# lim271/MultiOutputIHGP

Hardware: AMD Instinct MI355X
Metric: Kalman steps/sec (M outputs x T ticks) + NLL rel-err vs CPU oracle (higher is better)
Workload: dtype f32; 1 GPU; C3-filter: M=L=4096/GPU, T=10000, Matern-5/2 (matern52ss.h, d=3), fp32, filter+NLL; latents_per_gpu=4096, latents_total=4096, ticks=10000, state_dim=3, layout=segment-major [ceil(T/SEG)][L][SEG], SEG = 4 KB of ticks, HBM-resident

## Files before the change

multioutputihgp_amd/csrc/recursion.hip:

```cpp
#include "kernels_common.h"
#include <hip/hip_ext.h>

#ifndef MOIHGP_GENERIC_UNROLL
#define MOIHGP_GENERIC_UNROLL 4
#endif

namespace moihgp {
namespace {

template <typename T, int D, int CK>
struct FastConst {
    T a[D * D];
    T k[D];
    T g[CK * D];
    const T* sp;
    T pj[D * D];
};

template <typename T, int D, int CK, bool NLL, bool TAIL>
__device__ inline void replay_chunk(T* y, T* xs, const FastConst<T, D, CK>& c, size_t t0, size_t Tlen, double& acc, unsigned& nobs) {
    T part = 0;
#pragma unroll
    for (int k = 0; k < CK; k++) {
        const bool valid = !TAIL || (t0 + k) < Tlen;
// ... 417 lines not shown
            }
#pragma unroll
            for (int i = 0; i < D; i++) cc[i] = (double)read_lane(xs[i], jl);
            if (WRITE) {
#pragma unroll
                for (int k = 0; k < VPL; k++) lds[lane * (VPL + 1) + k] = pack<T>(&y[sg][k * EPV]);
                wave_lds_fence();
                T* po = orow + (size_t)sg * SEG + (size_t)lane * EPV;
#pragma unroll
                for (int i = 0; i < VPL; i++) {
                    const int q = i * 64 + lane;
                    if (sg < nfull || (size_t)sg * SEG + (size_t)q * EPV < Tlen) nt_store(lds[q + q / VPL], reinterpret_cast<V*>(po + (size_t)i * 64 * EPV));
                }
                wave_lds_fence();
            }
        }
    }
#pragma unroll
    for (int i = 0; i < D; i++) xout[i] = (T)cc[i];
    return true;
}

constexpr int kMaxSplit = 8;

template <typename T, int D, int CK, bool WRITE, bool NLL, int MINW, bool SPLIT, int DBG = 0>
__global__ void __launch_bounds__(SPLIT ? 64 * kMaxSplit : 64 * kWavesPerBlock, SPLIT ? 1 : MINW)
filter_scan_kernel(const T* __restrict__ Ty, size_t Ttot, size_t ld, size_t L, const T* __restrict__ cbT,
                   const double* __restrict__ cb64, const T* xin0 , T* x ,
                   T* __restrict__ yhat, double* __restrict__ nll, int nsplit, size_t Tslice,
                   int nbig ,
                   size_t ldo , int team ) {
    using V = typename VecOf<T>::type;
    using Lay = CB<D>;
    constexpr int EPV = 16 / sizeof(T);
    constexpr int VPL = CK / EPV;
    constexpr int NVP = 64 * (VPL + 1);
    static_assert(CK % EPV == 0 && CK <= 16, "CK must be a multiple of 16 bytes and fit the G table");
    extern __shared__ __attribute__((aligned(16))) unsigned char smem[];
    V (*lds_all)[NVP] = reinterpret_cast<V (*)[NVP]>(smem);
    constexpr int CR = D * D + D + 2;
    double (*carry)[CR] = reinterpret_cast<double (*)[CR]>(smem + (size_t)(SPLIT ? nsplit : kWavesPerBlock) * NVP * sizeof(V));

    const int lane = threadIdx.x & 63;
    const int wave = __builtin_amdgcn_readfirstlane(threadIdx.x >> 6);
    const size_t l = SPLIT ? (size_t)blockIdx.x : (size_t)blockIdx.x * kWavesPerBlock + wave;
    if (!SPLIT && l >= L) return;
    const size_t Tsl = SPLIT ? (wave < nbig ? Tslice : Tslice - 64 * CK) : 0;
    const size_t toff = SPLIT ? (wave < nbig ? (size_t)wave * Tslice : (size_t)nbig * Tslice + (size_t)(wave - nbig) * (Tslice - 64 * CK)) : 0;
    const size_t Tlen = SPLIT ? (toff >= Ttot ? 0 : ((Ttot - toff) < Tsl ? (Ttot - toff) : Tsl)) : Ttot;
    V* lds = lds_all[wave];

    const T* cb = cbT + l * Lay::SIZE;
    FastConst<T, D, CK> c;
#pragma unroll
    for (int i = 0; i < D * D; i++) c.a[i] = cb[Lay::A + i];
#pragma unroll
    for (int i = 0; i < D; i++) c.k[i] = cb[Lay::K + i];
#pragma unroll
    for (int i = 0; i < CK * D; i++) c.g[i] = cb[Lay::G + i];
    {
        T* spw = reinterpret_cast<T*>(smem + (size_t)(SPLIT ? nsplit : kWavesPerBlock) * NVP * sizeof(V) +
                                      (SPLIT ? (size_t)nsplit * CR * sizeof(double) : 0)) + (size_t)wave * (4 * D * D);
        if (lane < 4 * D * D) spw[lane] = cb[Lay::SP + lane];
        c.sp = spw;
        wave_lds_fence();
    }
#pragma unroll
    for (int i = 0; i < D * D; i++) c.pj[i] = cb[Lay::PJ + (lane & 15) * D * D + i];

    if (cb[Lay::SCANOK] == T(0)) return;
    const T* row = Ty + l * ld + toff;
    T* orow = WRITE ? yhat + l * ldo + toff : nullptr;
    T xin[D];
    double acc = 0.0;
    unsigned nobs = 0;
    size_t nobs_uniform = 0;

    bool team_done = false;
    if (SPLIT) {
        if (team) {
            unsigned char* tb = smem + (size_t)nsplit * NVP * sizeof(V) + (size_t)nsplit * CR * sizeof(double) + (((size_t)nsplit * 4 * D * D * sizeof(T) + 15) & ~(size_t)15);
            double (*e0all)[D] = reinterpret_cast<double (*)[D]>(tb);
            int* dirty = reinterpret_cast<int*>(tb + (size_t)kTeamMaxSegs * D * sizeof(double));
            if (threadIdx.x == 0) *dirty = 0;
            __syncthreads();
            team_done = team_slice<T, D, CK, WRITE, NLL>(row, orow, Tlen, toff, c, lds, lane, e0all, dirty, xin0 + l * D, xin, acc, nobs, nobs_uniform);
        }
    }
    if (SPLIT && !team_done) {
        if (wave < nsplit - 1) {
            T msl[D * D];
#pragma unroll
            for (int i = 0; i < D; i++) xin[i] = T(0);
            sweep<T, D, CK, false, false, true, 0>(row, nullptr, Tlen, xin, c, cb, lds, lane, acc, nobs, nobs_uniform, msl);
            if (lane == 0) {
#pragma unroll
                for (int i = 0; i < D * D; i++) carry[wave][i] = (double)msl[i];
#pragma unroll
                for (int i = 0; i < D; i++) carry[wave][D * D + i] = (double)xin[i];
            }
        }
        __syncthreads();
        double xc[D];
#pragma unroll
        for (int i = 0; i < D; i++) xc[i] = (double)xin0[l * D + i];
        for (int s = 0; s < wave; s++) {
            double xn[D];
#pragma unroll
            for (int i = 0; i < D; i++) {
                double a = carry[s][D * D + i];
#pragma unroll
                for (int j = 0; j < D; j++) a = fma(carry[s][i * D + j], xc[j], a);
                xn[i] = a;
            }
#pragma unroll
            for (int i = 0; i < D; i++) xc[i] = xn[i];
        }
#pragma unroll
        for (int i = 0; i < D; i++) xin[i] = (T)xc[i];
        acc = 0.0; nobs = 0; nobs_uniform = 0;
        __syncthreads();
    } else if (!SPLIT) {
#pragma unroll
        for (int i = 0; i < D; i++) xin[i] = xin0[l * D + i];
    }

    if (!team_done && (WRITE || NLL || !SPLIT || wave == nsplit - 1)) {
        T unused[D * D];
        sweep<T, D, CK, WRITE, NLL, false, DBG>(row, orow, Tlen, xin, c, cb, lds, lane, acc, nobs, nobs_uniform, unused);
    }

    if (NLL) {
#pragma unroll
        for (int o = 32; o > 0; o >>= 1) {
            acc += __shfl_xor(acc, o);
            nobs += __shfl_xor(nobs, o);
        }
    }
    const double* c64 = cb64 + l * Lay::SIZE;
    if (SPLIT) {
        if (NLL) {
            if (lane == 0) { carry[wave][D * D + D] = acc; carry[wave][D * D + D + 1] = (double)nobs_uniform + (double)nobs; }
            __syncthreads();
        }
        if (lane == 0 && wave == nsplit - 1) {
#pragma unroll
            for (int i = 0; i < D; i++) x[l * D + i] = xin[i];
        }
        if (NLL && lane == 0 && wave == 0) {
            double a = 0.0, n = 0.0;
            for (int s = 0; s < nsplit; s++) { a += carry[s][D * D + D]; n += carry[s][D * D + D + 1]; }
            nll[l] = 0.5 * (a / c64[Lay::S] + n * c64[Lay::LOGS]);
        }
    } else if (lane == 0) {
#pragma unroll
        for (int i = 0; i < D; i++) x[l * D + i] = xin[i];
        if (NLL) {
            double n = (double)nobs_uniform + (double)nobs;
            nll[l] = 0.5 * (acc / c64[Lay::S] + n * c64[Lay::LOGS]);
        }
    }
}

__global__ void __launch_bounds__(1024) nll_total_kernel(const double* __restrict__ nll, size_t L, double* __restrict__ total) {
    __shared__ double red[16];
    const int tid = threadIdx.x, lane = tid & 63, wave = tid >> 6;
    constexpr int kBatch = 8;
    double s = 0.0;
    for (size_t base = 0; base < L; base += (size_t)kBatch * 1024) {
        double v[kBatch];
#pragma unroll
        for (int j = 0; j < kBatch; j++) {
            const size_t i = base + (size_t)j * 1024 + tid;
            const double t = nll[i < L ? i : L - 1];
            v[j] = i < L ? t : 0.0;
        }
#pragma unroll
        for (int j = 0; j < kBatch; j++) s += v[j];
    }
#pragma unroll
    for (int o = 32; o > 0; o >>= 1) s += __shfl_xor(s, o);
    if (lane == 0) red[wave] = s;
    __syncthreads();
    if (tid == 0) {
        double t = 0.0;
        for (int w = 0; w < 16; w++) t += red[w];
        *total = t;
    }
}

template <typename T, int D, bool TILED = false>
__global__ void __launch_bounds__(64)
filter_seq_kernel(const T* __restrict__ Ty, size_t Tlen, size_t ld, size_t L, const T* __restrict__ cbT, const double* __restrict__ cb64,
                  const T* xin0, T* x, T* __restrict__ yhat, double* __restrict__ nll, size_t ldo) {
    using V = typename VecOf<T>::type;
    using Lay = CB<D>;
    constexpr int EPV = 16 / sizeof(T);
    constexpr size_t SEGT = 4096 / sizeof(T);
    auto at = [&](size_t l_, size_t t_, size_t ld_) { return TILED ? ((t_ / SEGT) * L + l_) * SEGT + t_ % SEGT : l_ * ld_ + t_; };
    const size_t l = (size_t)blockIdx.x * blockDim.x + threadIdx.x;
    if (l >= L) return;
    const T* cb = cbT + l * Lay::SIZE;
    if (cb[Lay::SCANOK] != T(0)) return;
    T a[D * D], kk[D], xs[D];
    for (int i = 0; i < D * D; i++) a[i] = cb[Lay::A + i];
    for (int i = 0; i < D; i++) { kk[i] = cb[Lay::K + i]; xs[i] = xin0[l * D + i]; }
    double acc = 0.0, n = 0.0;
    for (size_t tb = 0; tb < Tlen; tb += EPV) {
        T yv[EPV];
        unpack<T>(*reinterpret_cast<const V*>(Ty + at(l, tb, ld)), yv);
        for (int e = 0; e < EPV && tb + e < Tlen; e++) {
            const T yk = yv[e];
            const bool miss = (yk != yk);
            T hx = 0;
            for (int q = 0; q < D; q++) hx = fma(a[q], xs[q], hx);
            const T v = miss ? T(0) : yk - hx;
            if (!miss) { acc = fma((double)v, (double)v, acc); n += 1.0; }
            T xn[D];
            xn[0] = fma(kk[0], v, hx);
            for (int i = 1; i < D; i++) {
                T s = kk[i] * v;
                for (int q = 0; q < D; q++) s = fma(a[i * D + q], xs[q], s);
                xn[i] = s;
            }
            for (int i = 0; i < D; i++) xs[i] = xn[i];
            if (yhat) yhat[at(l, tb + e, ldo)] = xs[0];
        }
    }
    for (int i = 0; i < D; i++) x[l * D + i] = xs[i];
    if (nll) { const double* c64 = cb64 + l * Lay::SIZE; nll[l] = 0.5 * (acc / c64[Lay::S] + n * c64[Lay::LOGS]); }
}

#ifndef MOIHGP_FILTER_DMA
#define MOIHGP_FILTER_DMA 1
#endif
constexpr int kDmaRing32 = 8, kDmaWaves32 = 4;
constexpr int kDmaRing64 = 8, kDmaWaves64 = 3;
typedef __attribute__((address_space(3))) void lds_void_t;
typedef __attribute__((address_space(1))) const void glb_cvoid_t;
__device__ inline unsigned lds_addr_of(const void* p) { return (unsigned)(unsigned long long)(__attribute__((address_space(3))) const char*)p; }
template <int N> __device__ inline void wait_vmcnt() { asm volatile("s_waitcnt vmcnt(%0)" ::"n"(N) : "memory"); }

template <typename T> struct AsmVec;
template <> struct AsmVec<float> { using type = nt_f4; };
template <> struct AsmVec<double> { using type = nt_d2; };
__device__ inline void av_unpack(const nt_f4& v, float* o) { o[0] = v.x; o[1] = v.y; o[2] = v.z; o[3] = v.w; }
__device__ inline void av_unpack(const nt_d2& v, double* o) { o[0] = v.x; o[1] = v.y; }
__device__ inline nt_f4 av_pack(const float* i) { nt_f4 v = {i[0], i[1], i[2], i[3]}; return v; }
__device__ inline nt_d2 av_pack(const double* i) { nt_d2 v = {i[0], i[1]}; return v; }

template <typename AV>
__device__ inline void lds_read4(unsigned a0, unsigned a1, unsigned a2, unsigned a3, AV (&r)[4]) {
    asm volatile("ds_read_b128 %0, %4\n\tds_read_b128 %1, %5\n\tds_read_b128 %2, %6\n\tds_read_b128 %3, %7\n\ts_waitcnt lgkmcnt(0)"
                 : "=&v"(r[0]), "=&v"(r[1]), "=&v"(r[2]), "=&v"(r[3]) : "v"(a0), "v"(a1), "v"(a2), "v"(a3) : "memory");
}
template <typename AV>
__device__ inline void lds_write4(unsigned a0, unsigned a1, unsigned a2, unsigned a3, const AV (&r)[4]) {
    asm volatile("ds_write_b128 %4, %0\n\tds_write_b128 %5, %1\n\tds_write_b128 %6, %2\n\tds_write_b128 %7, %3"
                 :: "v"(r[0]), "v"(r[1]), "v"(r[2]), "v"(r[3]), "v"(a0), "v"(a1), "v"(a2), "v"(a3) : "memory");
}
template <typename AV>
__device__ inline void lds_read4_kb(unsigned a, AV (&r)[4]) {
    asm volatile("ds_read_b128 %0, %4\n\tds_read_b128 %1, %4 offset:1024\n\tds_read_b128 %2, %4 offset:2048\n\tds_read_b128 %3, %4 offset:3072\n\ts_waitcnt lgkmcnt(0)"
                 : "=&v"(r[0]), "=&v"(r[1]), "=&v"(r[2]), "=&v"(r[3]) : "v"(a) : "memory");
}
template <typename T, int N>
__device__ inline void lds_read_uniform(unsigned addr, T* out) {
    using AV = typename AsmVec<T>::type;
    constexpr int EPV = 16 / sizeof(T), NV = (N + EPV - 1) / EPV;
    static_assert(NV >= 1 && NV <= 5, "table row of 1..5 vectors");
    AV v[5];
    if constexpr (NV == 1) asm volatile("ds_read_b128 %0, %1\n\ts_waitcnt lgkmcnt(0)" : "=&v"(v[0]) : "v"(addr) : "memory");
    else if constexpr (NV == 2) asm volatile("ds_read_b128 %0, %2\n\tds_read_b128 %1, %2 offset:16\n\ts_waitcnt lgkmcnt(0)" : "=&v"(v[0]), "=&v"(v[1]) : "v"(addr) : "memory");
    else if constexpr (NV == 3) asm volatile("ds_read_b128 %0, %3\n\tds_read_b128 %1, %3 offset:16\n\tds_read_b128 %2, %3 offset:32\n\ts_waitcnt lgkmcnt(0)"
                                             : "=&v"(v[0]), "=&v"(v[1]), "=&v"(v[2]) : "v"(addr) : "memory");
    else if constexpr (NV == 4) asm volatile("ds_read_b128 %0, %4\n\tds_read_b128 %1, %4 offset:16\n\tds_read_b128 %2, %4 offset:32\n\tds_read_b128 %3, %4 offset:48\n\ts_waitcnt lgkmcnt(0)"
                                             : "=&v"(v[0]), "=&v"(v[1]), "=&v"(v[2]), "=&v"(v[3]) : "v"(addr) : "memory");
    else asm volatile("ds_read_b128 %0, %5\n\tds_read_b128 %1, %5 offset:16\n\tds_read_b128 %2, %5 offset:32\n\tds_read_b128 %3, %5 offset:48\n\tds_read_b128 %4, %5 offset:64\n\ts_waitcnt lgkmcnt(0)"
                      : "=&v"(v[0]), "=&v"(v[1]), "=&v"(v[2]), "=&v"(v[3]), "=&v"(v[4]) : "v"(addr) : "memory");
    T e[5 * EPV];
#pragma unroll
    for (int i = 0; i < NV; i++) av_unpack(v[i], &e[i * EPV]);
#pragma unroll
    for (int i = 0; i < N; i++) out[i] = e[i];
}

template <typename T, int D> constexpr bool kPackRows = sizeof(T) == 4 && D == 3;
typedef float f2 __attribute__((ext_vector_type(2)));
__device__ inline f2 pk_fma(f2 a, float b, f2 c) { const f2 bb = {b, b}; return __builtin_elementwise_fma(a, bb, c); }
struct Mat3Pk { float r[3]; f2 c[3]; };
__device__ inline Mat3Pk mat3pk(const float* m) {
    Mat3Pk o;
#pragma unroll
    for (int j = 0; j < 3; j++) { o.r[j] = m[j]; o.c[j].x = m[3 + j]; o.c[j].y = m[6 + j]; }
    return o;
}
__device__ inline void matvec_acc_pk(const Mat3Pk& m, const float* t, float& z0, f2& zz) {
#pragma unroll
    for (int j = 0; j < 3; j++) z0 = fma(m.r[j], t[j], z0);
#pragma unroll
    for (int j = 0; j < 3; j++) zz = pk_fma(m.c[j], t[j], zz);
}
__device__ inline unsigned pk_row_pos(unsigned e) { return e < 3 ? e : (e < 6 ? 4 + 2 * (e - 3) : 5 + 2 * (e - 6)); }
__device__ inline Mat3Pk lds_read_mat3pk(unsigned addr) {
    nt_f4 v0, v1, v2;
    asm volatile("ds_read_b128 %0, %3\n\tds_read_b128 %1, %3 offset:16\n\tds_read_b128 %2, %3 offset:32\n\ts_waitcnt lgkmcnt(0)"
                 : "=&v"(v0), "=&v"(v1), "=&v"(v2) : "v"(addr) : "memory");
    Mat3Pk o;
    o.r[0] = v0.x; o.r[1] = v0.y; o.r[2] = v0.z;
    o.c[0] = v1.xy; o.c[1] = v1.zw; o.c[2] = v2.xy;
    return o;
}
template <int CTRL, int ROW_MASK>
__device__ inline void dpp_level_pk(const Mat3Pk& m, float& z0, f2& zz) {
    const float t[3] = {dpp0<CTRL, ROW_MASK>(z0), dpp0<CTRL, ROW_MASK>(zz.x), dpp0<CTRL, ROW_MASK>(zz.y)};
    matvec_acc_pk(m, t, z0, zz);
}
template <int SPL>
__device__ inline void dpp_scan_dma_pk(float& z0, f2& zz, unsigned sp_addr, const Mat3Pk& m1 , const Mat3Pk& pj) {
    dpp_level_pk<DPP_ROW_SHR + 1, 0xF>(m1, z0, zz);
    dpp_level_pk<DPP_ROW_SHR + 2, 0xF>(lds_read_mat3pk(sp_addr + 1 * SPL), z0, zz);
    dpp_level_pk<DPP_ROW_SHR + 4, 0xF>(lds_read_mat3pk(sp_addr + 2 * SPL), z0, zz);
    dpp_level_pk<DPP_ROW_SHR + 8, 0xF>(lds_read_mat3pk(sp_addr + 3 * SPL), z0, zz);
    dpp_level_pk<DPP_ROW_BCAST15, 0x2>(pj, z0, zz);
    dpp_level_pk<DPP_ROW_BCAST15, 0x4>(pj, z0, zz);
    dpp_level_pk<DPP_ROW_BCAST15, 0x8>(pj, z0, zz);
}
template <int CK, bool NLL, bool TAIL>
__device__ inline void replay_chunk_pk(float* y, float& x0, f2& xx, const Mat3Pk& a, float k0, f2 kk, size_t t0, size_t Tlen, double& acc, unsigned& nobs) {
    float part = 0;
#pragma unroll
    for (int k = 0; k < CK; k++) {
        const bool valid = !TAIL || (t0 + k) < Tlen;
        float hx = 0;
        hx = fma(a.r[0], x0, hx); hx = fma(a.r[1], xx.x, hx); hx = fma(a.r[2], xx.y, hx);
        float v = y[k] - hx;
        if (TAIL) v = valid ? v : 0.f;
        if (NLL) {
            part = fma(v, v, part);
            if (TAIL) nobs += valid ? 1u : 0u;
        }
        const float xn0 = fma(k0, v, hx);
        const f2 vv = {v, v};
        f2 ss = kk * vv;
        ss = pk_fma(a.c[0], x0, ss); ss = pk_fma(a.c[1], xx.x, ss); ss = pk_fma(a.c[2], xx.y, ss);
        x0 = (TAIL && !valid) ? x0 : xn0;
        xx.x = (TAIL && !valid) ? xx.x : ss.x;
        xx.y = (TAIL && !valid) ? xx.y : ss.y;
        y[k] = x0;
    }
    if (NLL) acc += (double)part;
}

template <typename T, int D, int SPL >
__device__ inline void dpp_scan_dma(T* z, unsigned sp_addr, const T* pj) {
    T t[D], m[D * D];
    lds_read_uniform<T, D * D>(sp_addr + 0 * SPL, m);
#pragma unroll
    for (int i = 0; i < D; i++) t[i] = dpp0<DPP_ROW_SHR + 1, 0xF>(z[i]);
    matvec_acc<T, D>(m, t, z);
    lds_read_uniform<T, D * D>(sp_addr + 1 * SPL, m);
#pragma unroll
    for (int i = 0; i < D; i++) t[i] = dpp0<DPP_ROW_SHR + 2, 0xF>(z[i]);
    matvec_acc<T, D>(m, t, z);
    lds_read_uniform<T, D * D>(sp_addr + 2 * SPL, m);
#pragma unroll
    for (int i = 0; i < D; i++) t[i] = dpp0<DPP_ROW_SHR + 4, 0xF>(z[i]);
    matvec_acc<T, D>(m, t, z);
    lds_read_uniform<T, D * D>(sp_addr + 3 * SPL, m);
#pragma unroll
    for (int i = 0; i < D; i++) t[i] = dpp0<DPP_ROW_SHR + 8, 0xF>(z[i]);
    matvec_acc<T, D>(m, t, z);
#pragma unroll
    for (int i = 0; i < D; i++) t[i] = dpp0<DPP_ROW_BCAST15, 0x2>(z[i]);
    matvec_acc<T, D>(pj, t, z);
#pragma unroll
    for (int i = 0; i < D; i++) t[i] = dpp0<DPP_ROW_BCAST15, 0x4>(z[i]);
    matvec_acc<T, D>(pj, t, z);
#pragma unroll
    for (int i = 0; i < D; i++) t[i] = dpp0<DPP_ROW_BCAST15, 0x8>(z[i]);
    matvec_acc<T, D>(pj, t, z);
}

template <typename T, int D, int CK>
struct DmaConst {
    T a[D * D], k[D], g[CK * D];
    unsigned sp_addr;
    T pj[D * D];
};

template <typename T, int D, int CK, int SPL, bool NLL, int TAIL>
__device__ inline bool dma_segment(T* y, T* xin, const DmaConst<T, D, CK>& c, int lane, size_t t0, size_t Tlen, double& acc, unsigned& nobs) {
    if constexpr (kPackRows<T, D>) {
        float z0 = 0.f;
        f2 zz = {0.f, 0.f};
#pragma unroll
        for (int k = 0; k < CK; k++) {
            z0 = fma(c.g[k * 3], y[k], z0);
            const f2 gg = {c.g[k * 3 + 1], c.g[k * 3 + 2]};
            zz = pk_fma(gg, y[k], zz);
        }
        if (__any((z0 != z0) | (zz.x != zz.x) | (zz.y != zz.y))) return false;
        const Mat3Pk m1 = lds_read_mat3pk(c.sp_addr);
        {
            const float x0[3] = {(lane == 0) ? xin[0] : 0.f, (lane == 0) ? xin[1] : 0.f, (lane == 0) ? xin[2] : 0.f};
            matvec_acc_pk(m1, x0, z0, zz);
        }
        const Mat3Pk pj = mat3pk(c.pj), a = mat3pk(c.a);
        dpp_scan_dma_pk<SPL>(z0, zz, c.sp_addr, m1, pj);
        float xs0 = wave_shr1(z0, xin[0]);
        f2 xx = {wave_shr1(zz.x, xin[1]), wave_shr1(zz.y, xin[2])};
        const f2 kk = {c.k[1], c.k[2]};
        int jl = 63;
        if (TAIL == 1) {
            double part = 0.0; unsigned none = 0;
            replay_chunk_pk<CK, NLL, false>(y, xs0, xx, a, c.k[0], kk, t0, Tlen, part, none);
            const bool valid = t0 < Tlen;
            if (NLL) { acc += valid ? part : 0.0; nobs += valid ? (unsigned)CK : 0u; }
            jl = (int)((Tlen - 1 - (t0 - (size_t)lane * CK)) / CK);
        } else if (TAIL == 2) {
            replay_chunk_pk<CK, NLL, true>(y, xs0, xx, a, c.k[0], kk, t0, Tlen, acc, nobs);
            jl = (int)((Tlen - 1 - (t0 - (size_t)lane * CK)) / CK);
        } else {
            replay_chunk_pk<CK, NLL, false>(y, xs0, xx, a, c.k[0], kk, t0, Tlen, acc, nobs);
        }
        xin[0] = read_lane(xs0, jl); xin[1] = read_lane(xx.x, jl); xin[2] = read_lane(xx.y, jl);
        return true;
    }
    T z[D];
#pragma unroll
    for (int i = 0; i < D; i++) z[i] = T(0);
#pragma unroll
    for (int k = 0; k < CK; k++)
#pragma unroll
        for (int i = 0; i < D; i++) z[i] = fma(c.g[k * D + i], y[k], z[i]);
    bool bad = false;
#pragma unroll
    for (int i = 0; i < D; i++) bad |= (z[i] != z[i]);
    if (__any(bad)) return false;
    {
        T x0[D], m[D * D];
        lds_read_uniform<T, D * D>(c.sp_addr, m);
#pragma unroll
        for (int i = 0; i < D; i++) x0[i] = (lane == 0) ? xin[i] : T(0);
        matvec_acc<T, D>(m, x0, z);
    }
    dpp_scan_dma<T, D, SPL>(z, c.sp_addr, c.pj);
    T xs[D];
#pragma unroll
    for (int i = 0; i < D; i++) xs[i] = wave_shr1(z[i], xin[i]);
    FastConst<T, D, CK> fc;
#pragma unroll
    for (int i = 0; i < D * D; i++) fc.a[i] = c.a[i];
#pragma unroll
    for (int i = 0; i < D; i++) fc.k[i] = c.k[i];
    int jl = 63;
    if (TAIL == 1) {
        double part = 0.0; unsigned none = 0;
        replay_chunk<T, D, CK, NLL, false>(y, xs, fc, t0, Tlen, part, none);
        const bool valid = t0 < Tlen;
        if (NLL) { acc += valid ? part : 0.0; nobs += valid ? (unsigned)CK : 0u; }
        jl = (int)((Tlen - 1 - (t0 - (size_t)lane * CK)) / CK);
    } else if (TAIL == 2) {
        replay_chunk<T, D, CK, NLL, true>(y, xs, fc, t0, Tlen, acc, nobs);
        jl = (int)((Tlen - 1 - (t0 - (size_t)lane * CK)) / CK);
    } else {
        replay_chunk<T, D, CK, NLL, false>(y, xs, fc, t0, Tlen, acc, nobs);
    }
#pragma unroll
    for (int i = 0; i < D; i++) xin[i] = read_lane(xs[i], jl);
    return true;
}

template <typename T, int D, int CK, bool WRITE, bool NLL, int NP, int MINW, bool TILED = false>
__global__ void __launch_bounds__(64 * kWavesPerBlock, MINW)
filter_dma_kernel(const T* __restrict__ Ty, size_t Tlen, size_t ld, size_t L, const T* __restrict__ cbT, const double* __restrict__ cb64,
                  const T* xin0, T* x, T* __restrict__ yhat, double* __restrict__ nll, size_t ldo) {
    using Lay = CB<D>;
    using AV = typename AsmVec<T>::type;
    constexpr int EPV = 16 / sizeof(T);
    constexpr int VPL = CK / EPV;
    static_assert(VPL == 4, "a chunk is four 16-byte vectors in both precisions");
    constexpr int SEG = 64 * CK;
    constexpr int PT = 16 * CK;
    constexpr int SPL = ((D * D * (int)sizeof(T)) + 15) / 16 * 16;
    constexpr int WAVE_LDS = NP * 1024 + 4 * SPL;
    static_assert(NP >= 8 && NP <= 40, "ring of 8 .. 40 pieces");
    constexpr int WSTEADY = NP - 4 + (WRITE ? 4 : 0);
    extern __shared__ __attribute__((aligned(16))) unsigned char smem[];

    const int lane = threadIdx.x & 63;
    const int wave = __builtin_amdgcn_readfirstlane(threadIdx.x >> 6);
    const size_t l = (size_t)blockIdx.x * kWavesPerBlock + wave;
    if (l >= L) return;
    unsigned char* ring = smem + (size_t)wave * WAVE_LDS;
    const unsigned ring_addr = lds_addr_of(ring);
    const unsigned sp_addr = ring_addr + NP * 1024;
    const T* cb = cbT + l * Lay::SIZE;

    if (Tlen == 0) {
        if (lane == 0 && cb[Lay::SCANOK] != T(0)) {
#pragma unroll
            for (int i = 0; i < D; i++) x[l * D + i] = xin0[l * D + i];
            if (NLL) nll[l] = 0.0;
        }
        return;
    }
    const size_t nseg = (Tlen + SEG - 1) / SEG;
    const size_t nfullp = Tlen / PT;
    const unsigned jj = lane & 15, rr = lane >> 4;
    const unsigned sw = (jj ^ (jj >> 2)) & 3;
    const unsigned goff = (unsigned)(((lane & ~3) | ((lane & 3) ^ (((lane >> 2) ^ (lane >> 4)) & 3))) * 16);
    const unsigned char* rowb = TILED ? reinterpret_cast<const unsigned char*>(Ty) + l * 4096 : reinterpret_cast<const unsigned char*>(Ty + l * ld);
    const size_t seg_stride = TILED ? L * 4096 : 4096;
    const size_t lastv = ((Tlen - 1) / EPV) * 16;
    auto issue_piece = [&](size_t p, unsigned slot, bool inside) {
        lds_void_t* dst = (lds_void_t*)(ring + (size_t)slot * 1024);
        if (TILED) {
            if (inside) {
                __builtin_amdgcn_global_load_lds((glb_cvoid_t*)(rowb + (p >> 2) * seg_stride + (p & 3) * 1024 + goff), dst, 16, 0, 0);
            } else {
                const bool past = (p >> 2) >= nseg;
                const size_t ts = past ? nseg - 1 : (p >> 2);
                const unsigned lim = ts == nseg - 1 ? (unsigned)(lastv & 4095) : 4080u;
                unsigned o = past ? lim : (unsigned)(p & 3) * 1024 + goff;
                o = o < lim ? o : lim;
                __builtin_amdgcn_global_load_lds((glb_cvoid_t*)(rowb + ts * seg_stride + o), dst, 16, 0, 0);
            }
        } else if (inside) {
            __builtin_amdgcn_global_load_lds((glb_cvoid_t*)(rowb + p * 1024 + goff), dst, 16, 0, 0);
        } else {
            size_t o = p * 1024 + goff;
            o = o < lastv ? o : lastv;
            __builtin_amdgcn_global_load_lds((glb_cvoid_t*)(rowb + o), dst, 16, 0, 0);
        }
    };
    DmaConst<T, D, CK> c;
#pragma unroll
    for (int i = 0; i < D * D; i++) c.a[i] = cb[Lay::A + i];
#pragma unroll
    for (int i = 0; i < D; i++) c.k[i] = cb[Lay::K + i];
#pragma unroll
    for (int i = 0; i < CK * D; i++) c.g[i] = cb[Lay::G + i];
    c.sp_addr = sp_addr;
    const T scanok = cb[Lay::SCANOK];
    T xin[D];
#pragma unroll
    for (int i = 0; i < D; i++) xin[i] = xin0[l * D + i];
    if (nfullp >= (size_t)NP) {
#pragma unroll
        for (int i = 0; i < NP; i++) issue_piece((size_t)i, (unsigned)i, true);
    } else {
#pragma unroll
        for (int i = 0; i < NP; i++) issue_piece((size_t)i, (unsigned)i, false);
    }
#pragma unroll
    for (int i = 0; i < D * D; i++) c.pj[i] = cb[Lay::PJ + (lane & 15) * D * D + i];
    const T spv = cb[Lay::SP + (lane < 4 * D * D ? lane : 0)];

    double acc = 0.0;
    unsigned nobs = 0;
    size_t nobs_uniform = 0;
    unsigned char* orowb = WRITE ? (TILED ? reinterpret_cast<unsigned char*>(yhat) + l * 4096 : reinterpret_cast<unsigned char*>(yhat + l * ldo)) : nullptr;

    wait_vmcnt<NP - 4>();
    if (lane < 4 * D * D) {
        unsigned e = (unsigned)(lane % (D * D));
        if constexpr (kPackRows<T, D>) e = pk_row_pos(e);
        const unsigned a = sp_addr + (unsigned)(lane / (D * D)) * SPL + e * (unsigned)sizeof(T);
        if constexpr (sizeof(T) == 4) asm volatile("ds_write_b32 %0, %1" :: "v"(a), "v"(spv) : "memory");
        else asm volatile("ds_write_b64 %0, %1" :: "v"(a), "v"(spv) : "memory");
    }
    asm volatile("s_waitcnt lgkmcnt(0)" ::: "memory");

    constexpr bool RING4 = NP % 4 == 0;
    const size_t nin = nfullp / 4;
    const unsigned char* inb = rowb + (size_t)(NP / 4) * seg_stride;
    unsigned char* outb = orowb;
    const size_t nsweep = scanok == T(0) ? 0 : nseg;
    unsigned slot0 = 0;
    for (size_t seg = 0; seg < nsweep; seg++) {
        if (seg > 0) wait_vmcnt<WSTEADY>();
        const size_t tbase = seg * SEG;
        const size_t t0 = tbase + (size_t)lane * CK;
        unsigned sl = slot0 + rr;
        if constexpr (!RING4) sl = sl >= (unsigned)NP ? sl - NP : sl;
        const unsigned cbase = ring_addr + sl * 1024 + jj * 64;
        const unsigned ca0 = cbase + (sw << 4), ca1 = cbase + ((sw ^ 1u) << 4), ca2 = cbase + ((sw ^ 2u) << 4), ca3 = cbase + ((sw ^ 3u) << 4);
        bool done;
        {
            AV v[4];
            lds_read4<AV>(ca0, ca1, ca2, ca3, v);
            T y[CK];
#pragma unroll
            for (int k = 0; k < 4; k++) av_unpack(v[k], &y[k * EPV]);
            const bool full = tbase + SEG <= Tlen;
            if (full) {
                done = dma_segment<T, D, CK, SPL, NLL, 0>(y, xin, c, lane, t0, Tlen, acc, nobs);
                if (done) nobs_uniform += SEG;
            } else {
#pragma unroll
                for (int k = 0; k < CK; k++) y[k] = (t0 + k) < Tlen ? y[k] : T(0);
                if (Tlen % CK == 0) done = dma_segment<T, D, CK, SPL, NLL, 1>(y, xin, c, lane, t0, Tlen, acc, nobs);
                else done = dma_segment<T, D, CK, SPL, NLL, 2>(y, xin, c, lane, t0, Tlen, acc, nobs);
            }
            if (!done) {
#pragma unroll
                for (int k = 0; k < 4; k++) v[k] = av_pack(&y[k * EPV]);
                lds_write4<AV>(cbase, cbase + 16, cbase + 32, cbase + 48, v);
                asm volatile("s_waitcnt lgkmcnt(0)" ::: "memory");
                wave_lds_fence();
                T* chunk = reinterpret_cast<T*>(ring + (size_t)sl * 1024 + jj * 64);
                generic_segment<T, D, CK, NLL>(chunk, xin, cb, lane, t0, Tlen, acc, nobs);
                wave_lds_fence();
                if (WRITE) {
                    lds_read4<AV>(cbase, cbase + 16, cbase + 32, cbase + 48, v);
#pragma unroll
                    for (int k = 0; k < 4; k++) av_unpack(v[k], &y[k * EPV]);
                }
            }
            if (WRITE) {
#pragma unroll
                for (int k = 0; k < 4; k++) v[k] = av_pack(&y[k * EPV]);
                lds_write4<AV>(ca0, ca1, ca2, ca3, v);
            }
        }
        unsigned s1 = slot0 + 1, s2 = slot0 + 2, s3 = slot0 + 3;
        s1 = s1 >= (unsigned)NP ? s1 - NP : s1; s2 = s2 >= (unsigned)NP ? s2 - NP : s2; s3 = s3 >= (unsigned)NP ? s3 - NP : s3;
        if (WRITE) {
            AV o[4];
            const unsigned la = ring_addr + (unsigned)lane * 16;
            if constexpr (RING4) lds_read4_kb<AV>(la + slot0 * 1024, o);
            else lds_read4<AV>(la + slot0 * 1024, la + s1 * 1024, la + s2 * 1024, la + s3 * 1024, o);
            unsigned char* po = outb + goff;
            if (tbase + SEG <= Tlen) {
#pragma unroll
                for (int i = 0; i < 4; i++) __builtin_nontemporal_store(o[i], reinterpret_cast<AV*>(po + i * 1024));
            } else {
#pragma unroll
                for (int i = 0; i < 4; i++)
                    if (tbase * sizeof(T) + i * 1024 + goff < Tlen * sizeof(T)) __builtin_nontemporal_store(o[i], reinterpret_cast<AV*>(po + i * 1024));
            }
        }
        if (seg + 1 < nseg) {
            const size_t pn = 4 * seg + NP;
            if (RING4 && seg + NP / 4 < nin) {
                glb_cvoid_t* src = (glb_cvoid_t*)(inb + goff);
                lds_void_t* dst = (lds_void_t*)(ring + (size_t)slot0 * 1024);
                __builtin_amdgcn_global_load_lds(src, dst, 16, 0, 0);
                __builtin_amdgcn_global_load_lds(src, dst, 16, 1024, 0);
                __builtin_amdgcn_global_load_lds(src, dst, 16, 2048, 0);
                __builtin_amdgcn_global_load_lds(src, dst, 16, 3072, 0);
            } else if (pn + 4 <= nfullp) { issue_piece(pn + 0, slot0, true); issue_piece(pn + 1, s1, true); issue_piece(pn + 2, s2, true); issue_piece(pn + 3, s3, true); }
            else { issue_piece(pn + 0, slot0, false); issue_piece(pn + 1, s1, false); issue_piece(pn + 2, s2, false); issue_piece(pn + 3, s3, false); }
        }
        slot0 += 4; slot0 = slot0 >= (unsigned)NP ? slot0 - NP : slot0;
        inb += seg_stride;
        if (WRITE) outb += seg_stride;
    }
    wait_vmcnt<0>();

    if (scanok == T(0)) return;
    if (NLL) {
#pragma unroll
        for (int o = 32; o > 0; o >>= 1) {
            acc += __shfl_xor(acc, o);
            nobs += __shfl_xor(nobs, o);
        }
    }
    if (lane == 0) {
#pragma unroll
        for (int i = 0; i < D; i++) x[l * D + i] = xin[i];
        if (NLL) {
            const double* c64 = cb64 + l * Lay::SIZE;
            const double n = (double)nobs_uniform + (double)nobs;
            nll[l] = 0.5 * (acc / c64[Lay::S] + n * c64[Lay::LOGS]);
        }
    }
}

template <typename T, int D, int CK, int NP, int MINW, bool TILED = false>
int launch_filter_dma_t(const SweepIo& io, const T* cbT, const double* cb64, int n_unstable) {
    const size_t Tlen = io.T, ld = io.ld, L = io.L, ldo = io.ld_out;
    double* const nll = io.nll;
    const hipStream_t stream = io.stream;
    constexpr int SPL = ((D * D * (int)sizeof(T)) + 15) / 16 * 16;
    constexpr size_t smem = (size_t)kWavesPerBlock * (NP * 1024 + 4 * SPL);
    dim3 block(64 * kWavesPerBlock), grid((unsigned)((L + kWavesPerBlock - 1) / kWavesPerBlock));
    const T* ty = static_cast<const T*>(io.Ty);
    const T* xi = static_cast<const T*>(io.xin);
    T* xs = static_cast<T*>(io.x);
    T* yh = static_cast<T*>(io.yhat);
#define MOIHGP_DMA_LAUNCH(W_, N_)                                                                                                     \
    do {                                                                                                                              \
        auto kfn = filter_dma_kernel<T, D, CK, W_, N_, NP, MINW, TILED>;                                                              \
        if (smem > 65536) {                                                                                                           \
            static const hipError_t attr = hipFuncSetAttribute(reinterpret_cast<const void*>(kfn), hipFuncAttributeMaxDynamicSharedMemorySize, (int)smem); \
            if (attr != hipSuccess) { set_last_error("filter_dma_kernel: %zu bytes of LDS refused: %s", smem, hipGetErrorString(attr)); return 2; } \
        }                                                                                                                             \
        hipExtLaunchKernelGGL(kfn, grid, block, smem, stream, io.ev0, io.ev1, 0, ty, Tlen, ld, L, cbT, cb64, xi, xs, yh, nll, ldo);         \
    } while (0)
    if (yh && nll) MOIHGP_DMA_LAUNCH(true, true);
    else if (yh) MOIHGP_DMA_LAUNCH(true, false);
    else if (nll) MOIHGP_DMA_LAUNCH(false, true);
    else MOIHGP_DMA_LAUNCH(false, false);
#undef MOIHGP_DMA_LAUNCH
    if (n_unstable > 0)
        hipLaunchKernelGGL((filter_seq_kernel<T, D, TILED>), dim3((unsigned)((L + 63) / 64)), dim3(64), 0, stream, ty, Tlen, ld, L, cbT, cb64, xi, xs, yh, nll, ldo);
    if (io.total && nll) hipLaunchKernelGGL(nll_total_kernel, dim3(1), dim3(1024), 0, stream, nll, L, io.total);
    hipError_t e = hipGetLastError();
    if (e != hipSuccess) { set_last_error("filter_dma_kernel launch: %s", hipGetErrorString(e)); return 2; }
    return 0;
}

template <typename T, int D, int CK, int MINW, bool SPLIT>
int launch_filter_t(const SweepIo& io, const T* cbT, const double* cb64, int nsplit, size_t Tslice, int n_unstable, int nbig, int team_ok = 1) {
    const size_t Tlen = io.T, ld = io.ld, L = io.L, ldo = io.ld_out;
    double* const nll = io.nll;
    const hipStream_t stream = io.stream;
    dim3 block(SPLIT ? 64 * nsplit : 64 * kWavesPerBlock);
    dim3 grid(SPLIT ? (unsigned)L : (unsigned)((L + kWavesPerBlock - 1) / kWavesPerBlock));
    constexpr size_t tile = 64 * (CK / (16 / sizeof(T)) + 1) * 16;
    const size_t smem = (SPLIT ? (size_t)nsplit * (tile + (D * D + D + 2) * sizeof(double)) : (size_t)kWavesPerBlock * tile) +
                        (size_t)(SPLIT ? nsplit : kWavesPerBlock) * 4 * D * D * sizeof(T) +
                        (SPLIT ? (size_t)kTeamMaxSegs * D * sizeof(double) + 32 : 0);
    const int team = (SPLIT && team_ok && Tslice <= (size_t)kTeamSeg * 64 * CK && (Tlen + 64 * CK - 1) / (64 * CK) <= (size_t)kTeamMaxSegs) ? 1 : 0;
    const T* ty = static_cast<const T*>(io.Ty);
    const T* xi = static_cast<const T*>(io.xin);
    T* xs = static_cast<T*>(io.x);
    T* yh = static_cast<T*>(io.yhat);
    if (yh && nll)
        hipExtLaunchKernelGGL((filter_scan_kernel<T, D, CK, true, true, MINW, SPLIT>), grid, block, smem, stream, io.ev0, io.ev1, 0, ty, Tlen, ld, L, cbT, cb64, xi, xs, yh, nll, nsplit, Tslice, nbig, ldo, team);
    else if (yh)
        hipExtLaunchKernelGGL((filter_scan_kernel<T, D, CK, true, false, MINW, SPLIT>), grid, block, smem, stream, io.ev0, io.ev1, 0, ty, Tlen, ld, L, cbT, cb64, xi, xs, yh, nll, nsplit, Tslice, nbig, ldo, team);
    else if (nll)
        hipExtLaunchKernelGGL((filter_scan_kernel<T, D, CK, false, true, MINW, SPLIT>), grid, block, smem, stream, io.ev0, io.ev1, 0, ty, Tlen, ld, L, cbT, cb64, xi, xs, yh, nll, nsplit, Tslice, nbig, ldo, team);
    else
        hipExtLaunchKernelGGL((filter_scan_kernel<T, D, CK, false, false, MINW, SPLIT>), grid, block, smem, stream, io.ev0, io.ev1, 0, ty, Tlen, ld, L, cbT, cb64, xi, xs, yh, nll, nsplit, Tslice, nbig, ldo, team);
    if (n_unstable > 0)
        hipLaunchKernelGGL((filter_seq_kernel<T, D>), dim3((unsigned)((L + 63) / 64)), dim3(64), 0, stream, ty, Tlen, ld, L, cbT, cb64, xi, xs, yh, nll, ldo);
    if (io.total && nll) hipLaunchKernelGGL(nll_total_kernel, dim3(1), dim3(1024), 0, stream, nll, L, io.total);
    hipError_t e = hipGetLastError();
    if (e != hipSuccess) { set_last_error("filter_scan_kernel launch: %s", hipGetErrorString(e)); return 2; }
    return 0;
}

}

void launch_nll_total(const double* nll, size_t L, double* total, hipStream_t stream) {
    hipLaunchKernelGGL(nll_total_kernel, dim3(1), dim3(1024), 0, stream, nll, L, total);
}

void filter_split_plan(int dtype, size_t T, size_t L, int* nsplit, size_t* Tslice, int* nbig) {
    const size_t seg = 64 * (size_t)(dtype == 0 ? kChunk64 : kChunk32);
    *nsplit = 1; *Tslice = T; *nbig = 1;
    if (L == 0 || L > 512 || T < 2 * seg) return;
    size_t want = (2048 + L - 1) / L;
    if (want > (size_t)kMaxSplit) want = kMaxSplit;
    if (L > 256 && want > 4) want = 4;
    const size_t segs = (T + seg - 1) / seg;
    if (want > segs) want = segs;
    if (want < 2) return;
    const size_t per = (segs + want - 1) / want;
    const size_t big = segs - want * (per - 1);
    if (per == 1 && big < want) { *nsplit = (int)big; *Tslice = seg; *nbig = (int)big; return; }
    *nsplit = (int)want; *Tslice = per * seg; *nbig = (int)big;
}

template <typename T>
__global__ void __launch_bounds__(256) retile_kernel(const T* __restrict__ src, T* __restrict__ dst, size_t L, size_t Tlen, size_t ld, int to_tiled) {
    constexpr size_t SEGT = 4096 / sizeof(T);
    const size_t nseg = (Tlen + SEGT - 1) / SEGT;
    const size_t e = (size_t)blockIdx.x * 256 + threadIdx.x;
    if (e >= nseg * L * SEGT) return;
    const size_t sgi = e / (L * SEGT), l = (e / SEGT) % L, t = sgi * SEGT + e % SEGT;
    if (to_tiled) dst[e] = t < Tlen ? src[l * ld + t] : T(0);
    else if (t < Tlen) dst[l * ld + t] = src[e];
}
int launch_stream_retile(int dtype, const void* src, void* dst, size_t L, size_t T, size_t ld, int to_tiled, hipStream_t stream) {
    if (L == 0 || T == 0) return 0;
    const size_t segt = dtype == 0 ? 512 : 1024, n = (T + segt - 1) / segt * L * segt;
    const unsigned grid = (unsigned)((n + 255) / 256);
    if (dtype == 0) hipLaunchKernelGGL(retile_kernel<double>, dim3(grid), dim3(256), 0, stream, (const double*)src, (double*)dst, L, T, ld, to_tiled);
    else hipLaunchKernelGGL(retile_kernel<float>, dim3(grid), dim3(256), 0, stream, (const float*)src, (float*)dst, L, T, ld, to_tiled);
    hipError_t e = hipGetLastError();
    if (e != hipSuccess) { set_last_error("retile_kernel launch: %s", hipGetErrorString(e)); return 2; }
    return 0;
}

int launch_filter_stream_tiled(int d, const SweepIo& io, const double* cb64, const float* cb32, int n_unstable, int variant) {
    if (io.L == 0) return 0;
    const int dtype = io.dtype;
#ifdef MOIHGP_TUNING
    if (variant >= 20 && variant < 30 && d == 3) {
#define MOIHGP_DMA_PROBE_T(V_, NP_, MW_)                                                                                                \
        if (variant == V_) return dtype == 0 ? launch_filter_dma_t<double, 3, kChunk64, NP_, MW_, true>(io, cb64, cb64, n_unstable) \
                                             : launch_filter_dma_t<float, 3, kChunk32, NP_, MW_, true>(io, cb32, cb64, n_unstable)
        MOIHGP_DMA_PROBE_T(21, 9, 4); MOIHGP_DMA_PROBE_T(22, 12, 3); MOIHGP_DMA_PROBE_T(23, 16, 2); MOIHGP_DMA_PROBE_T(24, 8, 3); MOIHGP_DMA_PROBE_T(25, 12, 2);
#undef MOIHGP_DMA_PROBE_T
    }
#else
    (void)variant;
#endif
    if (dtype == 0) {
        if (d == 2) return launch_filter_dma_t<double, 2, kChunk64, kDmaRing64, kDmaWaves64, true>(io, cb64, cb64, n_unstable);
        return launch_filter_dma_t<double, 3, kChunk64, kDmaRing64, kDmaWaves64, true>(io, cb64, cb64, n_unstable);
    }
    if (d == 2) return launch_filter_dma_t<float, 2, kChunk32, kDmaRing32, kDmaWaves32, true>(io, cb32, cb64, n_unstable);
    return launch_filter_dma_t<float, 3, kChunk32, kDmaRing32, kDmaWaves32, true>(io, cb32, cb64, n_unstable);
}

int launch_filter_stream(int d, const SweepIo& io, const double* cb64, const float* cb32, int variant, int nsplit, size_t Tslice, int n_unstable, int nbig) {
    if (io.L == 0) return 0;
    const int dtype = io.dtype;
    if (nsplit > kMaxSplit) { set_last_error("nsplit > %d", kMaxSplit); return 1; }
    if (nbig <= 0 || nbig > nsplit) nbig = nsplit;
#define MOIHGP_FILTER_CASE(TT, DD, CKK, MW, CB)                                                                                   \
    do {                                                                                                                          \
        if (nsplit > 1) return launch_filter_t<TT, DD, CKK, 1, true>(io, CB, cb64, nsplit, Tslice, n_unstable, nbig); \
        return launch_filter_t<TT, DD, CKK, MW, false>(io, CB, cb64, 1, io.T, n_unstable, 1);                            \
    } while (0)
#ifdef MOIHGP_TUNING
    if (variant == 1 && dtype == 0 && d == 3) MOIHGP_FILTER_CASE(double, 3, kChunk64, 3, cb64);
    if (dtype == 1 && d == 3 && (variant == 2 || variant == 4 || variant == 6 || variant == 9)) {
        dim3 block(64 * kWavesPerBlock), grid((unsigned)((io.L + kWavesPerBlock - 1) / kWavesPerBlock));
        const size_t sm = (size_t)kWavesPerBlock * (64 * 5 * 16 + 36 * 4);
#define MOIHGP_PROBE(MW, DBG_) hipExtLaunchKernelGGL((filter_scan_kernel<float, 3, kChunk32, true, true, MW, false, DBG_>), grid, block, sm, io.stream, io.ev0, io.ev1, 0, \
                                                     (const float*)io.Ty, io.T, io.ld, io.L, cb32, cb64, (const float*)io.xin, (float*)io.x, (float*)io.yhat, io.nll, 1, io.T, 1, io.ld_out, 0)
        if (variant == 2) MOIHGP_PROBE(4, 2);
        else if (variant == 4) MOIHGP_PROBE(4, 4);
        else if (variant == 6) MOIHGP_PROBE(4, 6);
        else MOIHGP_PROBE(1, 1);
#undef MOIHGP_PROBE
        return 0;
    }
    if (variant == 1 && dtype == 1 && d == 3) MOIHGP_FILTER_CASE(float, 3, kChunk32, 1, cb32);
    if (variant >= 20 && variant < 30 && d == 3 && nsplit == 1) {
#define MOIHGP_DMA_PROBE(V_, NP_, MW_)                                                                                                  \
        if (variant == V_) return dtype == 0 ? launch_filter_dma_t<double, 3, kChunk64, NP_, MW_>(io, cb64, cb64, n_unstable) \
                                             : launch_filter_dma_t<float, 3, kChunk32, NP_, MW_>(io, cb32, cb64, n_unstable)
        MOIHGP_DMA_PROBE(20, 8, 4); MOIHGP_DMA_PROBE(21, 9, 4); MOIHGP_DMA_PROBE(22, 12, 3); MOIHGP_DMA_PROBE(23, 16, 2); MOIHGP_DMA_PROBE(24, 8, 3);
        MOIHGP_DMA_PROBE(25, 12, 2); MOIHGP_DMA_PROBE(26, 8, 2); MOIHGP_DMA_PROBE(27, 20, 2);
#undef MOIHGP_DMA_PROBE
    }
    if (variant == 10) variant = 0;
    else if (variant == 0) variant = -1;
#else
    if (variant != 0) { set_last_error("filter variant %d: tuning probes are compiled only with -DMOIHGP_TUNING", variant); return 1; }
    variant = -1;
#endif
    if (variant == -1 && nsplit == 1 && MOIHGP_FILTER_DMA) {
        if (dtype == 0) {
            if (d == 2) return launch_filter_dma_t<double, 2, kChunk64, kDmaRing64, kDmaWaves64>(io, cb64, cb64, n_unstable);
            return launch_filter_dma_t<double, 3, kChunk64, kDmaRing64, kDmaWaves64>(io, cb64, cb64, n_unstable);
        }
        if (d == 2) return launch_filter_dma_t<float, 2, kChunk32, kDmaRing32, kDmaWaves32>(io, cb32, cb64, n_unstable);
        return launch_filter_dma_t<float, 3, kChunk32, kDmaRing32, kDmaWaves32>(io, cb32, cb64, n_unstable);
    }
    if (dtype == 0) {
        if (d == 2) MOIHGP_FILTER_CASE(double, 2, kChunk64, 1, cb64);
        MOIHGP_FILTER_CASE(double, 3, kChunk64, 1, cb64);
    }
    if (d == 2) MOIHGP_FILTER_CASE(float, 2, kChunk32, 4, cb32);
    MOIHGP_FILTER_CASE(float, 3, kChunk32, 4, cb32);
#undef MOIHGP_FILTER_CASE
}

}
```

Measured before the change: 724.9 billion Kalman steps/s.

## Move chunk response coefficients to LDS and fuse broadcast scan levels into DPP FMAs

In the packed fp32 D=3 path, the per-chunk G coefficients (CK*3 floats) are no longer held in registers. They are written once per wave to LDS in a packed layout and read back with ds_read_b128 in groups, which frees VGPRs. The three row_bcast15 scan levels are rewritten as inline asm using v_fmac_f32_dpp, which removes the separate DPP move instructions. The row-shift levels use update_dpp with bound_ctrl, and the LDS read offsets become immediates. The trade-off is extra LDS traffic and waitcnt stalls in the hot segment loop, plus a slightly larger LDS footprint per wave.

```diff
diff --git a/multioutputihgp_amd/csrc/recursion.hip b/multioutputihgp_amd/csrc/recursion.hip
--- a/multioutputihgp_amd/csrc/recursion.hip
+++ b/multioutputihgp_amd/csrc/recursion.hip
@@ -743,29 +743,57 @@
     for (int j = 0; j < 3; j++) zz = pk_fma(m.c[j], t[j], zz);
 }
 __device__ inline unsigned pk_row_pos(unsigned e) { return e < 3 ? e : (e < 6 ? 4 + 2 * (e - 3) : 5 + 2 * (e - 6)); }
+template <int OFF = 0 >
 __device__ inline Mat3Pk lds_read_mat3pk(unsigned addr) {
     nt_f4 v0, v1, v2;
-    asm volatile("ds_read_b128 %0, %3\n\tds_read_b128 %1, %3 offset:16\n\tds_read_b128 %2, %3 offset:32\n\ts_waitcnt lgkmcnt(0)"
-                 : "=&v"(v0), "=&v"(v1), "=&v"(v2) : "v"(addr) : "memory");
+    asm volatile("ds_read_b128 %0, %3 offset:%4\n\tds_read_b128 %1, %3 offset:%5\n\tds_read_b128 %2, %3 offset:%6\n\ts_waitcnt lgkmcnt(0)"
+                 : "=&v"(v0), "=&v"(v1), "=&v"(v2) : "v"(addr), "n"(OFF), "n"(OFF + 16), "n"(OFF + 32) : "memory");
     Mat3Pk o;
     o.r[0] = v0.x; o.r[1] = v0.y; o.r[2] = v0.z;
     o.c[0] = v1.xy; o.c[1] = v1.zw; o.c[2] = v2.xy;
     return o;
 }
-template <int CTRL, int ROW_MASK>
+template <int CTRL>
+__device__ inline float dpp_shr0(float v) {
+    return __builtin_bit_cast(float, __builtin_amdgcn_update_dpp(0, __builtin_bit_cast(int, v), CTRL, 0xF, 0xF, true));
+}
+template <int CTRL>
+__device__ inline double dpp_shr0(double v) {
+    unsigned long long u = __builtin_bit_cast(unsigned long long, v);
+    unsigned lo = (unsigned)__builtin_amdgcn_update_dpp(0, (int)(unsigned)u, CTRL, 0xF, 0xF, true);
+    unsigned hi = (unsigned)__builtin_amdgcn_update_dpp(0, (int)(unsigned)(u >> 32), CTRL, 0xF, 0xF, true);
+    return __builtin_bit_cast(double, ((unsigned long long)hi << 32) | lo);
+}
+template <int CTRL>
 __device__ inline void dpp_level_pk(const Mat3Pk& m, float& z0, f2& zz) {
-    const float t[3] = {dpp0<CTRL, ROW_MASK>(z0), dpp0<CTRL, ROW_MASK>(zz.x), dpp0<CTRL, ROW_MASK>(zz.y)};
+    const float t[3] = {dpp_shr0<CTRL>(z0), dpp_shr0<CTRL>(zz.x), dpp_shr0<CTRL>(zz.y)};
     matvec_acc_pk(m, t, z0, zz);
 }
+#define MOIHGP_BCAST_LEVEL(MASK)                                               \
+    "v_fmac_f32_dpp %1, %0, %6 row_bcast:15 row_mask:" MASK " bank_mask:0xf\n\t"  \
+    "v_fmac_f32_dpp %2, %0, %7 row_bcast:15 row_mask:" MASK " bank_mask:0xf\n\t"  \
+    "v_fmac_f32_dpp %0, %0, %3 row_bcast:15 row_mask:" MASK " bank_mask:0xf\n\t"  \
+    "v_fmac_f32_dpp %2, %1, %9 row_bcast:15 row_mask:" MASK " bank_mask:0xf\n\t"  \
+    "v_fmac_f32_dpp %0, %1, %4 row_bcast:15 row_mask:" MASK " bank_mask:0xf\n\t"  \
+    "v_fmac_f32_dpp %1, %1, %8 row_bcast:15 row_mask:" MASK " bank_mask:0xf\n\t"  \
+    "v_fmac_f32_dpp %0, %2, %5 row_bcast:15 row_mask:" MASK " bank_mask:0xf\n\t"  \
+    "v_fmac_f32_dpp %1, %2, %10 row_bcast:15 row_mask:" MASK " bank_mask:0xf\n\t" \
+    "v_fmac_f32_dpp %2, %2, %11 row_bcast:15 row_mask:" MASK " bank_mask:0xf\n\t"
+__device__ inline void dpp_bcast_levels_pk(const Mat3Pk& pj, float& z0, f2& zz) {
+    float z1 = zz.x, z2 = zz.y;
+    asm("s_nop 1\n\t" MOIHGP_BCAST_LEVEL("0x2") MOIHGP_BCAST_LEVEL("0x4") MOIHGP_BCAST_LEVEL("0x8")
+        : "+v"(z0), "+v"(z1), "+v"(z2)
+        : "v"(pj.r[0]), "v"(pj.r[1]), "v"(pj.r[2]), "v"(pj.c[0].x), "v"(pj.c[0].y), "v"(pj.c[1].x), "v"(pj.c[1].y), "v"(pj.c[2].x), "v"(pj.c[2].y));
+    zz.x = z1; zz.y = z2;
+}
+#undef MOIHGP_BCAST_LEVEL
 template <int SPL>
 __device__ inline void dpp_scan_dma_pk(float& z0, f2& zz, unsigned sp_addr, const Mat3Pk& m1 , const Mat3Pk& pj) {
-    dpp_level_pk<DPP_ROW_SHR + 1, 0xF>(m1, z0, zz);
-    dpp_level_pk<DPP_ROW_SHR + 2, 0xF>(lds_read_mat3pk(sp_addr + 1 * SPL), z0, zz);
-    dpp_level_pk<DPP_ROW_SHR + 4, 0xF>(lds_read_mat3pk(sp_addr + 2 * SPL), z0, zz);
-    dpp_level_pk<DPP_ROW_SHR + 8, 0xF>(lds_read_mat3pk(sp_addr + 3 * SPL), z0, zz);
-    dpp_level_pk<DPP_ROW_BCAST15, 0x2>(pj, z0, zz);
-    dpp_level_pk<DPP_ROW_BCAST15, 0x4>(pj, z0, zz);
-    dpp_level_pk<DPP_ROW_BCAST15, 0x8>(pj, z0, zz);
+    dpp_level_pk<DPP_ROW_SHR + 1>(m1, z0, zz);
+    dpp_level_pk<DPP_ROW_SHR + 2>(lds_read_mat3pk<1 * SPL>(sp_addr), z0, zz);
+    dpp_level_pk<DPP_ROW_SHR + 4>(lds_read_mat3pk<2 * SPL>(sp_addr), z0, zz);
+    dpp_level_pk<DPP_ROW_SHR + 8>(lds_read_mat3pk<3 * SPL>(sp_addr), z0, zz);
+    dpp_bcast_levels_pk(pj, z0, zz);
 }
 template <int CK, bool NLL, bool TAIL>
 __device__ inline void replay_chunk_pk(float* y, float& x0, f2& xx, const Mat3Pk& a, float k0, f2 kk, size_t t0, size_t Tlen, double& acc, unsigned& nobs) {
@@ -798,19 +826,19 @@
     T t[D], m[D * D];
     lds_read_uniform<T, D * D>(sp_addr + 0 * SPL, m);
 #pragma unroll
-    for (int i = 0; i < D; i++) t[i] = dpp0<DPP_ROW_SHR + 1, 0xF>(z[i]);
+    for (int i = 0; i < D; i++) t[i] = dpp_shr0<DPP_ROW_SHR + 1>(z[i]);
     matvec_acc<T, D>(m, t, z);
     lds_read_uniform<T, D * D>(sp_addr + 1 * SPL, m);
 #pragma unroll
-    for (int i = 0; i < D; i++) t[i] = dpp0<DPP_ROW_SHR + 2, 0xF>(z[i]);
+    for (int i = 0; i < D; i++) t[i] = dpp_shr0<DPP_ROW_SHR + 2>(z[i]);
     matvec_acc<T, D>(m, t, z);
     lds_read_uniform<T, D * D>(sp_addr + 2 * SPL, m);
 #pragma unroll
-    for (int i = 0; i < D; i++) t[i] = dpp0<DPP_ROW_SHR + 4, 0xF>(z[i]);
+    for (int i = 0; i < D; i++) t[i] = dpp_shr0<DPP_ROW_SHR + 4>(z[i]);
     matvec_acc<T, D>(m, t, z);
     lds_read_uniform<T, D * D>(sp_addr + 3 * SPL, m);
 #pragma unroll
-    for (int i = 0; i < D; i++) t[i] = dpp0<DPP_ROW_SHR + 8, 0xF>(z[i]);
+    for (int i = 0; i < D; i++) t[i] = dpp_shr0<DPP_ROW_SHR + 8>(z[i]);
     matvec_acc<T, D>(m, t, z);
 #pragma unroll
     for (int i = 0; i < D; i++) t[i] = dpp0<DPP_ROW_BCAST15, 0x2>(z[i]);
@@ -823,9 +851,40 @@
     matvec_acc<T, D>(pj, t, z);
 }
 
+template <typename T, int D, int CK> constexpr int kDmaCoefBytes = kPackRows<T, D> ? CK * D * (int)sizeof(T) : 0;
+template <typename T, int D, int CK, int NP> constexpr int kDmaWaveLds = NP * 1024 + 4 * (((D * D * (int)sizeof(T)) + 15) / 16 * 16) + kDmaCoefBytes<T, D, CK>;
+__device__ inline unsigned pk_coef_pos(unsigned e) {
+    const unsigned k = e / 3, i = e % 3, q = k >> 2, kq = k & 3;
+    return q * 12 + (i == 0 ? kq : 4 + 2 * kq + (i - 1));
+}
+struct CoefGroup { nt_f4 r, c01, c23; };
+template <int OFF>
+__device__ inline void lds_read_coef(unsigned addr, CoefGroup (&g)[2]) {
+    asm volatile("ds_read_b128 %0, %6 offset:%7\n\tds_read_b128 %1, %6 offset:%7+16\n\tds_read_b128 %2, %6 offset:%7+32\n\t"
+                 "ds_read_b128 %3, %6 offset:%7+48\n\tds_read_b128 %4, %6 offset:%7+64\n\tds_read_b128 %5, %6 offset:%7+80\n\ts_waitcnt lgkmcnt(0)"
+                 : "=&v"(g[0].r), "=&v"(g[0].c01), "=&v"(g[0].c23), "=&v"(g[1].r), "=&v"(g[1].c01), "=&v"(g[1].c23) : "v"(addr), "n"(OFF) : "memory");
+}
+__device__ inline void coef_group_acc(const CoefGroup& g, const float* y, float& z0, f2& zz) {
+    z0 = fma(g.r.x, y[0], z0); zz = pk_fma(g.c01.xy, y[0], zz);
+    z0 = fma(g.r.y, y[1], z0); zz = pk_fma(g.c01.zw, y[1], zz);
+    z0 = fma(g.r.z, y[2], z0); zz = pk_fma(g.c23.xy, y[2], zz);
+    z0 = fma(g.r.w, y[3], z0); zz = pk_fma(g.c23.zw, y[3], zz);
+}
+template <int Q, int CK, int SPL>
+__device__ inline void coef_response(unsigned sp_addr, const float* y, float& z0, f2& zz) {
+    static_assert(CK % 8 == 0, "whole reads of the coefficient table");
+    if constexpr (Q < CK / 4) {
+        CoefGroup g[2];
+        lds_read_coef<4 * SPL + Q * 48>(sp_addr, g);
+        coef_group_acc(g[0], &y[4 * Q], z0, zz);
+        coef_group_acc(g[1], &y[4 * Q + 4], z0, zz);
+        coef_response<Q + 2, CK, SPL>(sp_addr, y, z0, zz);
+    }
+}
+
 template <typename T, int D, int CK>
 struct DmaConst {
-    T a[D * D], k[D], g[CK * D];
+    T a[D * D], k[D], g[kPackRows<T, D> ? 1 : CK * D];
     unsigned sp_addr;
     T pj[D * D];
 };
@@ -835,12 +894,7 @@
     if constexpr (kPackRows<T, D>) {
         float z0 = 0.f;
         f2 zz = {0.f, 0.f};
-#pragma unroll
-        for (int k = 0; k < CK; k++) {
-            z0 = fma(c.g[k * 3], y[k], z0);
-            const f2 gg = {c.g[k * 3 + 1], c.g[k * 3 + 2]};
-            zz = pk_fma(gg, y[k], zz);
-        }
+        coef_response<0, CK, SPL>(c.sp_addr, y, z0, zz);
         if (__any((z0 != z0) | (zz.x != zz.x) | (zz.y != zz.y))) return false;
         const Mat3Pk m1 = lds_read_mat3pk(c.sp_addr);
         {
@@ -925,7 +979,7 @@
     constexpr int SEG = 64 * CK;
     constexpr int PT = 16 * CK;
     constexpr int SPL = ((D * D * (int)sizeof(T)) + 15) / 16 * 16;
-    constexpr int WAVE_LDS = NP * 1024 + 4 * SPL;
+    constexpr int WAVE_LDS = kDmaWaveLds<T, D, CK, NP>;
     static_assert(NP >= 8 && NP <= 40, "ring of 8 .. 40 pieces");
     constexpr int WSTEADY = NP - 4 + (WRITE ? 4 : 0);
     extern __shared__ __attribute__((aligned(16))) unsigned char smem[];
@@ -981,8 +1035,10 @@
     for (int i = 0; i < D * D; i++) c.a[i] = cb[Lay::A + i];
 #pragma unroll
     for (int i = 0; i < D; i++) c.k[i] = cb[Lay::K + i];
-#pragma unroll
-    for (int i = 0; i < CK * D; i++) c.g[i] = cb[Lay::G + i];
+    if constexpr (!kPackRows<T, D>) {
+#pragma unroll
+        for (int i = 0; i < CK * D; i++) c.g[i] = cb[Lay::G + i];
+    }
     c.sp_addr = sp_addr;
     const T scanok = cb[Lay::SCANOK];
     T xin[D];
@@ -998,6 +1054,7 @@
 #pragma unroll
     for (int i = 0; i < D * D; i++) c.pj[i] = cb[Lay::PJ + (lane & 15) * D * D + i];
     const T spv = cb[Lay::SP + (lane < 4 * D * D ? lane : 0)];
+    const T gv = kPackRows<T, D> ? cb[Lay::G + (lane < CK * D ? lane : 0)] : T(0);
 
     double acc = 0.0;
     unsigned nobs = 0;
@@ -1005,12 +1062,17 @@
     unsigned char* orowb = WRITE ? (TILED ? reinterpret_cast<unsigned char*>(yhat) + l * 4096 : reinterpret_cast<unsigned char*>(yhat + l * ldo)) : nullptr;
 
     wait_vmcnt<NP - 4>();
+    if constexpr (kPackRows<T, D>) asm volatile("" :: "v"(spv), "v"(gv));
+    else asm volatile("" :: "v"(spv));
     if (lane < 4 * D * D) {
         unsigned e = (unsigned)(lane % (D * D));
         if constexpr (kPackRows<T, D>) e = pk_row_pos(e);
         const unsigned a = sp_addr + (unsigned)(lane / (D * D)) * SPL + e * (unsigned)sizeof(T);
         if constexpr (sizeof(T) == 4) asm volatile("ds_write_b32 %0, %1" :: "v"(a), "v"(spv) : "memory");
         else asm volatile("ds_write_b64 %0, %1" :: "v"(a), "v"(spv) : "memory");
+    }
+    if constexpr (kPackRows<T, D>) {
+        if (lane < CK * D) asm volatile("ds_write_b32 %0, %1" :: "v"(sp_addr + 4 * SPL + pk_coef_pos((unsigned)lane) * 4u), "v"(gv) : "memory");
     }
     asm volatile("s_waitcnt lgkmcnt(0)" ::: "memory");
 
@@ -1126,7 +1188,7 @@
     double* const nll = io.nll;
     const hipStream_t stream = io.stream;
     constexpr int SPL = ((D * D * (int)sizeof(T)) + 15) / 16 * 16;
-    constexpr size_t smem = (size_t)kWavesPerBlock * (NP * 1024 + 4 * SPL);
+    constexpr size_t smem = (size_t)kWavesPerBlock * kDmaWaveLds<T, D, CK, NP>;
     dim3 block(64 * kWavesPerBlock), grid((unsigned)((L + kWavesPerBlock - 1) / kWavesPerBlock));
     const T* ty = static_cast<const T*>(io.Ty);
     const T* xi = static_cast<const T*>(io.xin);
```

Result: no change. 720.5 billion Kalman steps/s (-0.6%).
